# dselivanov/rsparse

Hardware: AMD Instinct MI355X
Metric: als_iterations_per_sec (higher is better)
Workload: dtype f32 (Gram products of rows > 512 / <= 32 non-zeros as 2 x fp16 / 3 x bf16 split terms of the fp32 operands, fp32 accumulate; everything else fp32); 1 GPU; WRMF implicit ALS, CG(3), synthetic 10000000x1000000, 500155883 nnz, rank 128, lambda 0.1; survey_config=3, feedback=implicit, n_items=1000000, nnz=500155883, rank=128, solver=conjugate_gradient, cg_steps=3, parallelism=rows sharded x1, factors replicated

## Files before the change

rsparse_amd/csrc/wrmf_capi.cpp:

```cpp
#include "../../include/rsparse_wrmf_hip.h"

#include <cxxabi.h>

#include <algorithm>
#include <cfloat>
#include <cmath>
#include <cstdlib>
#include <cstring>
#include <functional>
#include <queue>
#include <string>
#include <vector>

#include "wrmf_internal.h"

using namespace rsparse_hip;

struct rsparse_hip_csc {
  DevCSC d;
  int device = 0;
};

namespace {

// ... 569 lines not shown
    hipError_t we = wave_cg ? launch_wide_cg_wave(a, implicit, kWideCgMaxLen, d.max_len > kWideCgMaxLen ? d.q_order : nullptr, 0, s)
                            : launch_als_wide(a, implicit, solver, g_ws.wide_m2, g_ws.wide_lu, s);
    if (we != hipSuccess) return hip_fail(we, wave_cg ? "launch_wide_cg_wave" : "launch_als_wide");
    if ((we = launch_sum_partials(g_ws.partials, wave_cg ? (size_t)grid_w : (size_t)grid, outw, s, g_ws.partials + g_ws.partial_slots)) != hipSuccess)
      return hip_fail(we, "launch_sum_partials");
    return RSPARSE_HIP_OK;
  }
  const bool cg = solver == RSPARSE_SOLVER_CONJUGATE_GRADIENT;
  const bool cgq = cg && use_cgq(rank, d_X, d_Y);
  QSchedule qs;
  qs.order = d.q_order;
  qs.cfg = d.q_cfg;
  qs.pair_first = d.q_pair_first;
  for (int b = 0; b < 7; b++) qs.off[b] = d.q_off[b];
  qs.team4_first = (implicit && bias && bias->gbias != 0.f) ? d.q_off[2] : d.q_team4_first;
  const bool ne_fine = implicit && padded_rank(rank) == 128;
  qs.ne_rows = ne_fine ? d.q_ne_rows : d.q_ne1_rows; qs.ne_ptr = ne_fine ? d.q_ne_ptr : d.q_ne1_ptr;
  qs.ne_wg = ne_fine ? d.q_ne_wg : d.q_ne1_wg; qs.ne_entries = d.q_ne_entries;
  qs.ne_split_rows = d.q_ne_split_rows; qs.ne_split_ptr = d.q_ne_split_ptr; qs.ne_nsplit = d.q_ne_nsplit;
  const bool cg_mf = cgq && implicit && !bias && cg_mf_supported(rank, implicit) && d.q_order && d.q_off[1] > d.q_n_nec;
  if (cg_mf) {
    qs.ne_rows = d.q_nec_rows; qs.ne_ptr = d.q_nec_ptr; qs.ne_wg = d.q_nec_wg; qs.ne_entries = d.q_nec_entries;
    qs.ne_split_rows = d.q_nec_split_rows; qs.ne_split_ptr = d.q_nec_split_ptr; qs.ne_nsplit = d.q_nec_nsplit;
    qs.mf_rows = d.q_order + d.q_n_nec;
    qs.mf_n = d.q_off[1] - d.q_n_nec;
  }
  const bool chol_mf = chol_mf_supported(rank) && !cg && solver == RSPARSE_SOLVER_CHOLESKY && !bias && d.q_order && ne_supported(rank) &&
                       use_cgq(rank, d_X, d_Y) && d.q_lr_first > d.q_off[1];
  const int mf_first = d.q_off[1];
  const int n_mf = chol_mf ? d.q_lr_first - mf_first : 0;
// ... 1182 lines not shown
```

rsparse_amd/csrc/wrmf_cgp.hip:

```cpp
#include "wrmf_internal.h"
#include "wrmf_device.h"

namespace rsparse_hip {
namespace {

using namespace dev;

typedef float f32x2 __attribute__((ext_vector_type(2)));
typedef float f32x4 __attribute__((ext_vector_type(4)));
typedef _Float16 f16x2 __attribute__((ext_vector_type(2)));
typedef _Float16 f16x8 __attribute__((ext_vector_type(8)));

constexpr float kCgTolP = 1e-10f;
constexpr int kPairMaxSweeps = 4;

__device__ __forceinline__ float p_row16_sum(float v) {
  v += dpp<0xB1>(v);
  v += dpp<0x4E>(v);
  v += dpp<0x141>(v);
  v += dpp<0x140>(v);
  return v;
}
__device__ __forceinline__ float p_row16_max(float v) {
  v = fmaxf(v, dpp<0xB1>(v));
// ... 8 lines not shown
  return __uint_as_float(r[0]) + __uint_as_float(r[1]);
}
__device__ __forceinline__ int p_scale_exp(float vmax) {
  const int eb = (int)((__float_as_uint(vmax) >> 23) & 0xffu);
  return min(253, max(1, 267 - eb));
}
__device__ __forceinline__ void p_split(const float x0, const float x1, unsigned& hi, unsigned& lo) {
  const f32x2 v = {x0, x1};
  const f16x2 h = __builtin_convertvector(v, f16x2);
  const f32x2 r = v - __builtin_convertvector(h, f32x2);
  const f16x2 l = __builtin_convertvector(r, f16x2);
  hi = __builtin_bit_cast(unsigned, h);
  lo = __builtin_bit_cast(unsigned, l);
}

struct PairSmem {
  static constexpr int KP = 128, ps = KP + 8, os = KP + 4;
  static constexpr size_t bytes = (size_t)2 * 8 * ps * 2 + (size_t)8 * os * 4 + (size_t)4 * 64 * 4 + 16;
};

template <bool GB, bool KFULL = false>
__global__ __launch_bounds__(256, 2) void als_cgp_kernel(AlsArgs a, const int32_t* __restrict__ rows, int n_rows, int iters,
                                                        size_t loss_slot0) {
  constexpr int KP = 128, RPN = 8, VW = 4, NV = 2, NQ = 8;
  using SM = PairSmem;
  extern __shared__ __attribute__((aligned(16))) char smem[];
  _Float16* sPh = reinterpret_cast<_Float16*>(smem);
  _Float16* sPl = sPh + 8 * SM::ps;
  float* sOut = reinterpret_cast<float*>(sPl + 8 * SM::ps);
  float* sTsv = sOut + 8 * SM::os;
  const int tid = threadIdx.x, lane = tid & 63, wv = rfl(tid >> 6);
  const int g = lane >> 4, i = lane & 15, H = lane >> 5, g2 = g & 1;
  const int k = KFULL ? KP : a.k;
  const float gbias = GB ? a.gbias : 0.f, ltgt = GB ? a.loss_tgt_const : 1.f;
  for (int e = tid; e < 4 * 64; e += 256) sTsv[e] = 0.f;
  f16x8 gAh[2][4], gAl[2][4];
  float ginv;
  {
    const int m = lane & 15, kb = lane >> 4;
    float gmax = 0.f;
#pragma unroll
    for (int t = 0; t < 2; t++)
#pragma unroll
      for (int ks = 0; ks < 4; ks++)
#pragma unroll
        for (int e = 0; e < 8; e++) {
          const int r = 32 * wv + 16 * t + m, c = 32 * ks + 8 * kb + e;
          {
            const float gv = a.XtX[(size_t)min(r, k - 1) * k + min(c, k - 1)];
            gmax = fmaxf(gmax, fabsf(gv) * ((r < k && c < k) ? 1.f : 0.f));
          }
// ... 5 lines not shown
#pragma unroll
    for (int t = 0; t < 2; t++)
#pragma unroll
      for (int ks = 0; ks < 4; ks++) {
        unsigned hi[4], lo[4];
#pragma unroll
        for (int e = 0; e < 8; e += 2) {
          const int r = 32 * wv + 16 * t + m, c = 32 * ks + 8 * kb + e;
          const float g0v = a.XtX[(size_t)min(r, k - 1) * k + min(c, k - 1)];
          const float g0 = g0v * ((r < k && c < k) ? 1.f : 0.f);
          const float g1v = a.XtX[(size_t)min(r, k - 1) * k + min(c + 1, k - 1)];
          const float g1 = g1v * ((r < k && c + 1 < k) ? 1.f : 0.f);
          p_split(g0 * gs, g1 * gs, hi[e / 2], lo[e / 2]);
        }
        const uint4 h4 = {hi[0], hi[1], hi[2], hi[3]}, l4 = {lo[0], lo[1], lo[2], lo[3]};
        gAh[t][ks] = __builtin_bit_cast(f16x8, h4);
        gAl[t][ks] = __builtin_bit_cast(f16x8, l4);
      }
  }
  __syncthreads();
  float* tacc = sTsv + wv * 64 + 16 * H;
  float* tcur = tacc + 32;
  const int col = 2 * wv + H;
  double wloss = 0.0;
  const int wave_global = blockIdx.x * 4 + wv, total_waves = gridDim.x * 4;
  auto ridx = [&](const int itn) { return (wave_global + itn * total_waves) * 2 + H; };
  int row_c = 0, p1_c = 0, p2_c = 0, row_n = 0;
  if (iters > 0 && ridx(0) < n_rows) {
    row_c = rows[ridx(0)];
    p1_c = a.col_ptrs[row_c];
    p2_c = a.col_ptrs[row_c + 1];
  }
  if (iters > 1 && ridx(1) < n_rows) row_n = rows[ridx(1)];

  int idn[NQ];
  float cvn[NQ], cln = 0.f;
#pragma unroll
  for (int q = 0; q < NQ; q++) {
    idn[q] = 0;
    cvn[q] = 0.f;
  }
  auto request_indices = [&](const bool valid, const int np1, const int ncnt) {
#pragma unroll
    for (int q = 0; q < NQ; q++) {
      const int s = 2 * q + g2;
      const int j = (valid && s < ncnt) ? np1 + s : 0;
      idn[q] = a.row_idx[j];
      cvn[q] = a.vals[j];
    }
    cln = a.vals[(valid && i < ncnt) ? np1 + i : 0];
  };
  auto settle_indices = [&]() {
    asm volatile("" : "+v"(idn[0]), "+v"(idn[1]), "+v"(idn[2]), "+v"(idn[3]), "+v"(idn[4]), "+v"(idn[5]), "+v"(idn[6]), "+v"(idn[7]));
    asm volatile("" : "+v"(cvn[0]), "+v"(cvn[1]), "+v"(cvn[2]), "+v"(cvn[3]), "+v"(cvn[4]), "+v"(cvn[5]), "+v"(cvn[6]), "+v"(cvn[7]), "+v"(cln));
  };
  if constexpr (KFULL) {
    request_indices(iters > 0 && ridx(0) < n_rows, p1_c, p2_c - p1_c);
    settle_indices();
  }

  for (int it = 0; it < iters; ++it) {
    const bool have = ridx(it) < n_rows;
    const int row = have ? row_c : 0, p1 = have ? p1_c : 0, p2 = have ? p2_c : 0;
    {
      int p1_n = 0, p2_n = 0, row_nn = 0;
      if (it + 1 < iters && ridx(it + 1) < n_rows) {
        p1_n = a.col_ptrs[row_n];
        p2_n = a.col_ptrs[row_n + 1];
      }
      if (it + 2 < iters && ridx(it + 2) < n_rows) row_nn = rows[ridx(it + 2)];
      row_c = row_n;
      p1_c = p1_n;
      p2_c = p2_n;
      row_n = row_nn;
    }
    const int cnt = p2 - p1;
    float* yrow = a.Y + (size_t)row * k;
    const bool live = have && (GB || cnt > 0);
    if (have && !live) {
      for (int e = lane & 31; e < k; e += 32) yrow[e] = 0.f;
    }
    const bool blk2 = max(__builtin_amdgcn_readlane(cnt, 0), __builtin_amdgcn_readlane(cnt, 32)) > 8;

    float x[RPN], r[RPN], p[RPN], ap[RPN];
    auto load_warm_start = [&]() {
#pragma unroll
      for (int b = 0; b < NV; b++) {
        const int off = b * 16 * VW + i * VW;
        float4 pc = make_float4(0.f, 0.f, 0.f, 0.f);
        if (have && off < k) pc = *reinterpret_cast<const float4*>(yrow + off);
        const float* pf = reinterpret_cast<const float*>(&pc);
#pragma unroll
        for (int c = 0; c < VW; c++) x[b * VW + c] = pf[c];
      }
    };
    if constexpr (KFULL) load_warm_start();
    float xt[NQ][RPN], cv[NQ];
    {
      int id[NQ];
#pragma unroll
      for (int q = 0; q < NQ; q++) {
        if constexpr (KFULL) {
          id[q] = idn[q];
          cv[q] = cvn[q];
        } else {
          const int s = 2 * q + g2;
          const int j = s < cnt ? p1 + s : 0;
          id[q] = 0;
          cv[q] = 0.f;
          if (q < 4 || blk2) {
            id[q] = a.row_idx[j];
            cv[q] = a.vals[j];
          }
        }
      }
#pragma unroll
      for (int q = 0; q < NQ; q++) {
        const bool in = 2 * q + g2 < cnt;
        id[q] = in ? id[q] : 0;
        cv[q] = in ? cv[q] : 0.f;
      }
#pragma unroll
      for (int q = 0; q < NQ; q++) {
        const bool in = 2 * q + g2 < cnt;
        const float* src = in ? a.X + (size_t)id[q] * k : a.zero_row;
#pragma unroll
        for (int b = 0; b < NV; b++) {
          const int off = b * 16 * VW + i * VW;
          if constexpr (KFULL) {
            float4 pc = make_float4(0.f, 0.f, 0.f, 0.f);
            if (q < 4 || blk2) pc = *reinterpret_cast<const float4*>(src + off);
            const float* pf = reinterpret_cast<const float*>(&pc);
#pragma unroll
            for (int c = 0; c < VW; c++) xt[q][b * VW + c] = pf[c];
          } else {
            float4 pc = make_float4(0.f, 0.f, 0.f, 0.f);
            if (q < 4 || blk2) pc = *reinterpret_cast<const float4*>(src + min(off, k - VW));
            const float* pf = reinterpret_cast<const float*>(&pc);
#pragma unroll
            for (int c = 0; c < VW; c++) xt[q][b * VW + c] = off < k ? pf[c] : 0.f;
          }
        }
      }
    }
    float cl;
    if constexpr (KFULL) cl = (g2 == 0 && i < cnt) ? cln : 0.f;
    else cl = (g2 == 0 && i < cnt) ? a.vals[p1 + i] : 0.f;

    if constexpr (!KFULL) load_warm_start();

    auto sweep = [&](const float(&v)[RPN], const int mode, float(&out)[RPN], float& loss_out) {
      float acc[RPN];
#pragma unroll
      for (int rr = 0; rr < RPN; rr++) acc[rr] = 0.f;
      float vinv = 0.f;
      if (mode != 2) {
        float vmax = 0.f;
#pragma unroll
        for (int rr = 0; rr < RPN; rr++) vmax = fmaxf(vmax, fabsf(v[rr]));
        vmax = p_row16_max(vmax);
        const int ve = p_scale_exp(vmax);
        const float vs = __uint_as_float((unsigned)ve << 23);
// ... 8 lines not shown
          const int off = col * SM::ps + g2 * 16 * VW + i * VW;
          *reinterpret_cast<uint2*>(sPh + off) = make_uint2(h0, h1);
          *reinterpret_cast<uint2*>(sPl + off) = make_uint2(l0, l1);
        }
        __syncthreads();
        f32x4 d0[2], d1[2];
#pragma unroll
        for (int t = 0; t < 2; t++) d0[t] = d1[t] = f32x4{0.f, 0.f, 0.f, 0.f};
        const int nb = (lane & 7) * SM::ps + 8 * (lane >> 4);
#pragma unroll
        for (int ks = 0; ks < 4; ks++) {
          const f16x8 bh = *reinterpret_cast<const f16x8*>(sPh + nb + 32 * ks);
          const f16x8 bl = *reinterpret_cast<const f16x8*>(sPl + nb + 32 * ks);
#pragma unroll
          for (int t = 0; t < 2; t++) {
            d0[t] = __builtin_amdgcn_mfma_f32_16x16x32_f16(gAh[t][ks], bh, d0[t], 0, 0, 0);
            d1[t] = __builtin_amdgcn_mfma_f32_16x16x32_f16(gAh[t][ks], bl, d1[t], 0, 0, 0);
            d1[t] = __builtin_amdgcn_mfma_f32_16x16x32_f16(gAl[t][ks], bh, d1[t], 0, 0, 0);
          }
        }
        if ((lane & 15) < 8) {
#pragma unroll
          for (int t = 0; t < 2; t++) {
            const f32x4 d = (d0[t] + d1[t]) * ginv;
            *reinterpret_cast<f32x4*>(sOut + (lane & 15) * SM::os + 32 * wv + 16 * t + 4 * (lane >> 4)) = d;
          }
        }
      }
      float lacc = 0.f;
      if (mode != 2) {
        float* trec = (mode == 0 ? tacc : tcur) + g2;
#pragma unroll
        for (int q0 = 0; q0 < NQ; q0 += 4) {
          if (q0 == 0 || blk2) {
            float t[4];
            f32x2 s2[4];
#pragma unroll
            for (int u = 0; u < 4; u++) s2[u] = f32x2{0.f, 0.f};
#pragma unroll
            for (int rr = 0; rr < RPN; rr += 2) {
              const f32x2 va = {v[rr], v[rr + 1]};
#pragma unroll
              for (int u = 0; u < 4; u++) {
                const f32x2 xa = {xt[q0 + u][rr], xt[q0 + u][rr + 1]};
                s2[u] = __builtin_elementwise_fma(xa, va, s2[u]);
              }
            }
#pragma unroll
            for (int u = 0; u < 4; u++) t[u] = s2[u].x + s2[u].y;
#pragma unroll
            for (int u = 0; u < 4; u++) t[u] += dpp<0xB1>(t[u]);
#pragma unroll
            for (int u = 0; u < 4; u++) t[u] += dpp<0x4E>(t[u]);
#pragma unroll
            for (int u = 0; u < 4; u++) t[u] += dpp<0x141>(t[u]);
#pragma unroll
            for (int u = 0; u < 4; u++) t[u] += dpp<0x140>(t[u]);
#pragma unroll
            for (int u = 0; u < 4; u++) {
              const int q = q0 + u;
              const float c = cv[q];
              trec[2 * q] = t[u];
              const float w = mode == 0 ? c - (c - 1.f) * (GB ? t[u] + gbias : t[u]) : (c - 1.f) * t[u];
#pragma unroll
              for (int rr = 0; rr < RPN; rr++) acc[rr] = fmaf(w, xt[q][rr], acc[rr]);
            }
          }
        }
      } else {
        wave_sync();
        const float t = tacc[i];
        const float dd = ltgt - t;
        lacc = p_pair_sum(p_row16_sum((g2 == 0 && i < cnt) ? cl * dd * dd : 0.f));
      }
      if (mode != 2) {
        __syncthreads();
        const float f = g2 == 0 ? vinv : 0.f;
#pragma unroll
        for (int b = 0; b < NV; b++) {
          const f32x4 o = *reinterpret_cast<const f32x4*>(sOut + col * SM::os + b * 16 * VW + i * VW);
#pragma unroll
          for (int c = 0; c < VW; c++) acc[b * VW + c] = fmaf(f, o[c], acc[b * VW + c]);
        }
#pragma unroll
        for (int rr = 0; rr < RPN; rr++) out[rr] = p_pair_sum(acc[rr]);
        if constexpr (GB) {
          if (mode == 0) {
#pragma unroll
// ... 8 lines not shown
        }
      } else {
        loss_out = lacc;
      }
    };
    auto dot16 = [&](const float(&u)[RPN], const float(&w)[RPN]) {
      float s = 0.f;
#pragma unroll
      for (int rr = 0; rr < RPN; rr++) s = fmaf(u[rr], w[rr], s);
      return p_row16_sum(s);
    };

    float dummy = 0.f;
    sweep(x, 0, r, dummy);
    if constexpr (KFULL)
      request_indices(it + 1 < iters && ridx(it + 1) < n_rows, p1_c, p2_c - p1_c);
#pragma unroll
    for (int rr = 0; rr < RPN; rr++) p[rr] = r[rr];
    float rsold = dot16(r, r);
    bool conv = !live;
    for (int itc = 0; itc < a.cg_steps; ++itc) {
      sweep(p, 1, ap, dummy);
      const float pap = dot16(p, ap);
      const float alpha = conv ? 0.f : (float)((double)rsold / (double)pap);
      wave_sync();
      if (g2 == 0) tacc[i] = fmaf(alpha, tcur[i], tacc[i]);
      wave_sync();
#pragma unroll
      for (int rr = 0; rr < RPN; rr++) {
        x[rr] = fmaf(alpha, p[rr], x[rr]);
        r[rr] = fmaf(-alpha, ap[rr], r[rr]);
      }
      const float rsnew = dot16(r, r);
      if (!conv) {
        if (rsnew < kCgTolP) {
          conv = true;
        } else {
          const float beta = (float)((double)rsnew / (double)rsold);
#pragma unroll
          for (int rr = 0; rr < RPN; rr++) p[rr] = fmaf(p[rr], beta, r[rr]);
          rsold = rsnew;
// ... 18 lines not shown
#pragma unroll
            for (int c = 0; c < VW; c++) pf[c] = x[b * VW + c];
            *reinterpret_cast<float4*>(yrow + off) = pc;
          }
        }
      }
    }
  }
  const double other = __shfl(wloss, 32);
  if (lane == 0) a.loss_partials[loss_slot0 + (size_t)blockIdx.x * 4 + wv] = wloss + other;
}

}

bool cgp_supported(int k, bool implicit) { return implicit && k > 64 && k <= 128 && k % 4 == 0; }

int cgp_grid(int n_rows) {
  if (n_rows <= 0) return 0;
  const long pairs = ((long)n_rows + 1) / 2;
  long per_wave = 32;
  const long spread = 4L * 512;
  if (pairs < spread * per_wave) per_wave = (pairs + spread - 1) / spread;
  if (per_wave < 1) per_wave = 1;
  return (int)((pairs + 4 * per_wave - 1) / (4 * per_wave));
}

hipError_t launch_als_cgp(const AlsArgs& a, const int32_t* rows, int n_rows, size_t loss_slot0, hipStream_t s,
                          hipEvent_t* ev_slot) {
  const int grid = cgp_grid(n_rows);
  if (grid <= 0) return hipSuccess;
  const long pairs = ((long)n_rows + 1) / 2;
  const int iters = (int)((pairs + (long)grid * 4 - 1) / ((long)grid * 4));
  const bool gb = a.gbias != 0.f;
  auto k0 = als_cgp_kernel<false, false>;
  auto k0f = als_cgp_kernel<false, true>;
  auto k1 = als_cgp_kernel<true, false>;
  const bool full = !gb && a.k == 128;
  const void* fn = gb ? reinterpret_cast<const void*>(k1) : (full ? reinterpret_cast<const void*>(k0f) : reinterpret_cast<const void*>(k0));
  hipError_t err = hipFuncSetAttribute(fn, hipFuncAttributeMaxDynamicSharedMemorySize, (int)PairSmem::bytes);
  if (err != hipSuccess) return err;
  (void)ev_slot;
  if (gb) hipLaunchKernelGGL(k1, dim3(grid), dim3(256), PairSmem::bytes, s, a, rows, n_rows, iters, loss_slot0);
  else if (full) hipLaunchKernelGGL(k0f, dim3(grid), dim3(256), PairSmem::bytes, s, a, rows, n_rows, iters, loss_slot0);
  else hipLaunchKernelGGL(k0, dim3(grid), dim3(256), PairSmem::bytes, s, a, rows, n_rows, iters, loss_slot0);
  return hipGetLastError();
}

}
```

rsparse_amd/csrc/wrmf_cgq.hip:

```cpp
#include <algorithm>

#include "wrmf_internal.h"
#include "wrmf_device.h"

namespace rsparse_hip {
namespace {

using namespace dev;

typedef float f32x2 __attribute__((ext_vector_type(2)));

constexpr int kGvFirstMinCapq = 16;
constexpr int kStreamPrefixQ = 4;
constexpr int kIdxPrefetchMaxWpr = 2;

constexpr float kCgTolQ = 1e-10f;
constexpr int kMaxSavedSweeps = 4;

template <int KP>
struct QG {
  static constexpr int RPN = KP / 16;
  static constexpr int VW = RPN >= 4 ? 4 : RPN;
  static constexpr int NV = RPN / VW;
  __device__ static __forceinline__ int elem(int i, int r) { return (r / VW) * (16 * VW) + i * VW + (r % VW); }
// ... 56 lines not shown
__device__ __forceinline__ void split_f16(const float x0, const float x1, unsigned& hi, unsigned& lo) {
  const f32x2 v = {x0, x1};
  const f16x2 h = __builtin_convertvector(v, f16x2);
  const f32x2 r = v - __builtin_convertvector(h, f32x2);
  const f16x2 l = __builtin_convertvector(r, f16x2);
  hi = __builtin_bit_cast(unsigned, h);
  lo = __builtin_bit_cast(unsigned, l);
}
__device__ __forceinline__ float row16_max(float v) {
  v = fmaxf(v, dpp<0xB1>(v));
  v = fmaxf(v, dpp<0x4E>(v));
  v = fmaxf(v, dpp<0x141>(v));
  v = fmaxf(v, dpp<0x140>(v));
  return v;
}

__device__ __forceinline__ unsigned lds_addr(const void* p) {
  return (unsigned)(reinterpret_cast<uintptr_t>(p));
}
__device__ __forceinline__ void dma4(const void* g, unsigned lds_base) {
  asm volatile("s_mov_b32 m0, %1\n\ts_nop 0\n\tglobal_load_lds_dword %0, off" : : "v"(g), "s"(lds_base) : "memory", "m0");
}
__device__ __forceinline__ void wait_vm0() { asm volatile("s_waitcnt vmcnt(0)" ::: "memory"); }

template <int KP, int CAPQ, int WAVES, int WPR, int STREAM, bool IMPLICIT, int DMF = 0>
struct QSmem {
  static constexpr size_t gram_floats = (IMPLICIT && DMF != 1) ? (size_t)KP * KP : 0;
  static constexpr size_t vec_floats = IMPLICIT ? (size_t)WAVES * KP : 0;
  static constexpr size_t red_floats = WPR > 1 ? (size_t)2 * WAVES * KP + 2 * WAVES : 0;
  static constexpr bool cv_lds = !STREAM && CAPQ * (KP / 16) > 128;
  static constexpr size_t tsv_floats = (STREAM && !IMPLICIT) ? 0 : (size_t)WAVES * (cv_lds ? 3 : 2) * CAPQ * 4;
  static constexpr size_t pre_floats = STREAM ? (size_t)WAVES * kStreamPrefixQ * 4 * KP : 0;
  static constexpr int dmf_ps = KP + 8, dmf_os = KP + 4;
  static constexpr size_t dmf_floats = DMF ? (size_t)WAVES * dmf_ps + (size_t)WAVES * dmf_os : 0;
  static constexpr size_t pfx_floats =
      (!STREAM && WPR > kIdxPrefetchMaxWpr && (CAPQ == 16 || CAPQ == 20)) ? (size_t)WAVES * 2 * CAPQ * 4 : 0;
  static constexpr size_t wl_floats = cv_lds ? (size_t)WAVES * 2 : 0;
  static constexpr size_t xs_floats = cv_lds ? (size_t)WAVES * KP : 0;
// ... 837 lines not shown
};
constexpr int cfg_of_kp(int KP) { return KP == 64 ? 1 : 0; }
constexpr int kTeam4Waves = 4, kTeam4Capq = 20;
static_assert(kTeam4Max == kTeam4Waves * kTeam4Capq * 4, "wrmf_internal.h's split and the kernel's capacity");
constexpr bool team4_split(int KP, bool GB) { return KP == 128 && !GB; }
int team4_first(const QSchedule& q) { return std::min(std::max(q.team4_first, q.off[1]), q.off[2]); }

template <int KP, int WAVES, int CAPQ, int WPR, int STREAM, bool IMPLICIT, bool GB, int DMF = 0, bool KFULL = false>
hipError_t launch_bucket(const AlsArgs& a, const int32_t* rows, int n_rows, int grid, size_t slot0, hipStream_t s,
                         hipEvent_t* ev_slot) {
  if (n_rows <= 0) return hipSuccess;
  constexpr bool kDmfGeometry = IMPLICIT && KP == 128 && WAVES == 4 && WPR == 1 && (CAPQ == 8 || CAPQ == 16) && STREAM == 0;
  if constexpr (kDmfGeometry && !DMF) {
    return launch_bucket<KP, WAVES, CAPQ, WPR, STREAM, IMPLICIT, GB, CAPQ == 8 ? 1 : 2>(a, rows, n_rows, grid, slot0, s, ev_slot);
  } else {
    if constexpr (!KFULL && STREAM == 0) {
      if (a.k == KP)
        return launch_bucket<KP, WAVES, CAPQ, WPR, STREAM, IMPLICIT, GB, DMF, true>(a, rows, n_rows, grid, slot0, s, ev_slot);
    }
    constexpr int TEAMS = WAVES / WPR;
    auto kern = als_cgq_kernel<KP, CAPQ, WAVES, WPR, STREAM, IMPLICIT, DMF, GB, KFULL>;
    const size_t lds = QSmem<KP, CAPQ, WAVES, WPR, STREAM, IMPLICIT, DMF>::bytes;
    hipError_t err = hipFuncSetAttribute(reinterpret_cast<const void*>(kern),
                                         hipFuncAttributeMaxDynamicSharedMemorySize, (int)lds);
    if (err != hipSuccess) return err;
    const int total_teams = grid * TEAMS;
    const int rpt = (n_rows + total_teams - 1) / total_teams;
    prof_note(ev_slot, reinterpret_cast<const void*>(kern));
    hipLaunchKernelGGL(kern, dim3(grid), dim3(WAVES * 64), lds, s, a, rows, n_rows, rpt, slot0);
    return hipGetLastError();
  }
// ... 24 lines not shown
int g_launch_mode = 2;
int concurrent_buckets() { return g_launch_mode; }

size_t bucket_slots(const QSchedule& q, int b, int k, bool implicit) {
  const int cfg = cfg_of_kp(padded_rank(k));
  const BucketDef d = kBuckets[cfg][b];
  if (d.wpr <= 0) return 0;
  if (d.stream && ne_supported(k)) return (size_t)(q.ne_entries + q.ne_nsplit) + (size_t)(q.mf_n > 0 ? cg_mf_loss_slots(q.mf_n) : 0);
  const int rows = q.off[b + 1] - q.off[b];
  if (b == 1 && padded_rank(k) == 128) {
    const int split = team4_first(q);
    return (size_t)cgq_bucket_grid(split - q.off[b], b, cfg) * d.waves + (size_t)cgq_team4_grid(q.off[b + 1] - split) * kTeam4Waves;
  }
  if (b == kNB - 1 && rows > 0 && cgp_supported(k, implicit)) {
    const int split = std::min(std::max(q.pair_first, q.off[b]), q.off[b + 1]);
    return (size_t)cgq_bucket_grid(split - q.off[b], b, cfg) * d.waves + (size_t)cgp_grid(q.off[b + 1] - split) * 4;
  }
  return (size_t)cgq_bucket_grid(rows, b, cfg) * d.waves;
}

template <int KP, int CFG, bool IMPLICIT, bool GB>
hipError_t launch_all(const AlsArgs& a, const QSchedule& q, hipStream_t s, hipEvent_t* ev) {
  hipError_t err;
  size_t slot = 0;
  const int cmode = ev ? 0 : concurrent_buckets();
  const bool overlap = cmode != 0;
  bool forked = false;
  if (overlap) {
    if ((err = g_bs.ensure()) != hipSuccess) return err;
  }
#define RSP_BUCKET(B)                                                                                       \
// ... 43 lines not shown
          return hipErrorInvalidValue;                                                                      \
        } else if constexpr (B == 1 && team4_split(KP, GB)) {                                              \
           \
          const int first = q.off[B], split = team4_first(q);                                               \
          const int n_main = split - first, n_t4 = q.off[B + 1] - split;                                    \
          const int g_main = cgq_bucket_grid(n_main, B, CFG);                                               \
          if ((err = launch_bucket<KP, D.waves, D.capq, D.wpr, D.stream, IMPLICIT, GB>(a, q.order + first, n_main, g_main, slot, \
                                                                                  bs, ev ? ev + B : nullptr)) != hipSuccess) \
            return err;                                                                                     \
          if ((err = launch_bucket<KP, kTeam4Waves, kTeam4Capq, kTeam4Waves, 0, IMPLICIT, GB>(              \
                   a, q.order + split, n_t4, cgq_team4_grid(n_t4), slot + (size_t)g_main * D.waves, bs,     \
                   n_main > 0 ? nullptr : (ev ? ev + B : nullptr))) != hipSuccess)                          \
            return err;                                                                                     \
        } else if (B == kNB - 1 && cgp_supported(a.k, IMPLICIT)) {                    \
           \
          const int first = q.off[B], split = std::min(std::max(q.pair_first, first), q.off[B + 1]);         \
          const int n_main = split - first, n_pair = q.off[B + 1] - split;                                   \
          const int g_main = cgq_bucket_grid(n_main, B, CFG);                                                \
          if ((err = launch_bucket<KP, D.waves, D.capq, D.wpr, D.stream, IMPLICIT, GB>(a, q.order + first, n_main, g_main, slot, \
                                                                                  bs, ev ? ev + B : nullptr)) != hipSuccess) \
            return err;                                                                                     \
          if ((err = launch_als_cgp(a, q.order + split, n_pair, slot + (size_t)g_main * D.waves, bs,          \
                                    n_main > 0 ? nullptr : (ev ? ev + B : nullptr))) != hipSuccess)           \
            return err;                                                                                     \
        } else if ((err = launch_bucket<KP, D.waves, D.capq, D.wpr, D.stream, IMPLICIT, GB>(a, q.order + q.off[B], n, grid, slot, \
                                                                                bs, ev ? ev + B : nullptr)) != hipSuccess) \
          return err;                                                                                       \
        if (side) {                                                                                         \
          if ((err = hipEventRecord(g_bs.done[B], bs)) != hipSuccess) return err;                           \
          if ((err = hipStreamWaitEvent(s, g_bs.done[B], 0)) != hipSuccess) return err;                     \
        }                                                                                                   \
      }                                                                                                     \
      slot += bucket_slots(q, B, a.k, IMPLICIT);                                                             \
    }                                                                                                       \
  }
  RSP_BUCKET(0)
  RSP_BUCKET(1)
// ... 72 lines not shown
```

rsparse_amd/csrc/wrmf_device.h:

```cpp
#pragma once
#include <hip/hip_runtime.h>

namespace rsparse_hip {
namespace dev {

__device__ __forceinline__ void wave_sync() {
  __builtin_amdgcn_fence(__ATOMIC_RELEASE, "wavefront");
  __builtin_amdgcn_wave_barrier();
  __builtin_amdgcn_fence(__ATOMIC_ACQUIRE, "wavefront");
}

__device__ __forceinline__ float readlane_f(float v, int l) {
  return __int_as_float(__builtin_amdgcn_readlane(__float_as_int(v), l));
}
__device__ __forceinline__ int rfl(int v) { return __builtin_amdgcn_readfirstlane(v); }

template <int CTRL>
__device__ __forceinline__ float dpp(float v) {
  return __int_as_float(__builtin_amdgcn_update_dpp(0, __float_as_int(v), CTRL, 0xf, 0xf, true));
}

template <int E>
__device__ __forceinline__ void fnma_row_bcast(float& acc, const float u, const float l) {
  asm("v_fmac_f32_dpp %0, -%1, %2 row_newbcast:%3 row_mask:0xf bank_mask:0xf" : "+v"(acc) : "v"(u), "v"(l), "n"(E));
}
__device__ __forceinline__ void dpp_ready(float& a) { asm("s_nop 1" : "+v"(a)); }
__device__ __forceinline__ void dpp_ready(float& a, float& b) { asm("s_nop 1" : "+v"(a), "+v"(b)); }
__device__ __forceinline__ void dpp_ready(float& a, float& b, float& c, float& d) {
  asm("s_nop 1" : "+v"(a), "+v"(b), "+v"(c), "+v"(d));
}
// ... 156 lines not shown
```

rsparse_amd/csrc/wrmf_internal.h:

```cpp
#pragma once
#include <hip/hip_runtime.h>
#include <cstdint>
#include <string>

namespace rsparse_hip {

struct DevCSC {
  int n_rows = 0;
  int n_cols = 0;
  int64_t nnz = 0;
  const int32_t* col_ptrs = nullptr;
  const int32_t* row_idx = nullptr;
  const float* vals = nullptr;
  int32_t* long_rows = nullptr;
  int n_long = 0;
  int short_max = 0;
  int max_len = 0;
  int32_t* q_order = nullptr;
  int q_off[7] = {0, 0, 0, 0, 0, 0, 0};
  int q_cfg = 0;
  int q_pair_first = 0;
  int q_team4_first = 0;
  int64_t q_nnz[6] = {0, 0, 0, 0, 0, 0};
  int64_t* q_stream_off = nullptr;
// ... 79 lines not shown
  const int32_t* ne_segs;
  float* ne_seg_scratch;
  int* ne_seg_flags;
  int ne_chol;
  int ne_chol_min;
  const unsigned* ne_stats;
  const float* mf_XtX;
  const unsigned* wave_stats;
};

struct QSchedule {
  const int32_t* order;
  int off[7];
  int pair_first;
  int team4_first;
  int cfg;
  const int32_t* ne_rows;
  const int32_t* ne_ptr;
  int ne_wg;
  int ne_entries;
  const int32_t* ne_split_rows;
  const int32_t* ne_split_ptr;
  int ne_nsplit;
  const int32_t* mf_rows = nullptr;
  int mf_n = 0;
};
int cgq_default_cfg();
void cgq_set_launch_mode(int mode);
int cgq_num_buckets();
int cgq_bucket_wpr(int cfg, int b);
int cgq_bucket_capq(int cfg, int b);
int cgq_bucket_waves(int cfg, int b);
int cgq_bucket_stream(int cfg, int b);
int cgq_bucket_grid(int n_rows, int bucket, int cfg);
constexpr int kTeam4Max = 320;
int cgq_team4_grid(int n_rows);
int cgq_bucket_of(int len, int cfg);
size_t cgq_loss_slots(const QSchedule& q, int k, bool implicit);
bool cgp_supported(int k, bool implicit);
int cgp_grid(int n_rows);
hipError_t launch_als_cgp(const AlsArgs& a, const int32_t* rows, int n_rows, size_t loss_slot0, hipStream_t s,
                          hipEvent_t* ev_slot);
bool ne_supported(int k);
constexpr int kNeMinLen = 512;
constexpr int kNeMaxSeg = 16;
constexpr int kNeMaxSegTotal = 1024;
constexpr int kNeSegFloats = 4 * (11 * 16 * 64 + 128 + 2);
hipError_t launch_ne_stats(const float* X, int64_t nx, const float* vals, int64_t nnz, unsigned* stats, hipStream_t s,
                           const float* absmax_hint = nullptr, const unsigned* cached_vstats = nullptr,
                           unsigned* save_vstats = nullptr);
struct QSchedule;
hipError_t launch_als_ne(const AlsArgs& a, const QSchedule& q, bool implicit, double* row_loss, hipStream_t s,
                         hipEvent_t* ev_slot = nullptr);
hipError_t launch_gb_row_terms(const AlsArgs& a, const int32_t* rows, int n, float* out, int32_t* slot_of_row, hipStream_t s);
hipError_t launch_als_cgq(const AlsArgs& a, const QSchedule& q, bool implicit, hipStream_t s, hipEvent_t* ev = nullptr);

// ... 139 lines not shown
```

rsparse_amd/csrc/wrmf_ne.hip:

```cpp
#include <type_traits>
#include <utility>

#include "wrmf_internal.h"
#include "wrmf_device.h"
#include "wrmf_ldlt.h"

namespace rsparse_hip {
namespace {

using namespace dev;

typedef float f32x16 __attribute__((ext_vector_type(16)));
typedef float f32x2 __attribute__((ext_vector_type(2)));
typedef __bf16 bf16x2 __attribute__((ext_vector_type(2)));
typedef __bf16 bf16x8 __attribute__((ext_vector_type(8)));
typedef unsigned u32x4 __attribute__((ext_vector_type(4)));

constexpr float kCgTolNe = 1e-10f;
constexpr int kStepNnz = 16;

struct NeMfmaOp { int slot, m, R, C, pa, pb; };
struct NeUnit { int kind, t, pair; };

template <int KP, int NS, bool IMPLICIT, bool SYM = false, bool QUAD = false>
// ... 110 lines not shown
  static constexpr int GROUP = NI / LOADERS + (LOADERS == 1 ? 2 : 1);
  static constexpr int RING_BYTES = D * SLOT_BYTES + IDXR * 256;
  static constexpr int TLD = 33;
  static constexpr int A_FLOATS = NT * 32 * TLD;
  static constexpr int G_FLOATS = IMPLICIT && !QUAD ? A_FLOATS : 0;
  static constexpr int YB = QUAD ? 4 : 8;
  static constexpr int V_FLOATS = 4 * KP  + 2 * NB * NB * 32  +
                                  4 * KP  + 256  +
                                  YB * KP + 4 * YB  + 64 ;
  static constexpr int BYTES = NRING * RING_BYTES + (A_FLOATS + G_FLOATS + V_FLOATS) * 4;
  static_assert(BYTES <= (QUAD ? 80 : 160) * 1024, "LDS budget");
  static_assert((D - 2) * GROUP <= 63, "vmcnt is a 6-bit field");
  __host__ __device__ static constexpr int tile(int R, int C) { return R * (R + 1) / 2 + C; }
};

__device__ __forceinline__ unsigned lds_addr(const void* p) {
  return (unsigned)(reinterpret_cast<uintptr_t>(p));
}

__device__ __forceinline__ void dma16(const void* g, unsigned lds_base) {
  asm volatile("s_mov_b32 m0, %1\n\ts_nop 0\n\tglobal_load_lds_dwordx4 %0, off" : : "v"(g), "s"(lds_base) : "memory", "m0");
}
__device__ __forceinline__ void dma4(const void* g, unsigned lds_base) {
  asm volatile("s_mov_b32 m0, %1\n\ts_nop 0\n\tglobal_load_lds_dword %0, off" : : "v"(g), "s"(lds_base) : "memory", "m0");
}
template <int N>
__device__ __forceinline__ void wait_vm() {
  asm volatile("s_waitcnt vmcnt(%0)" ::"n"(N) : "memory");
}
__device__ __forceinline__ int sload(const int* p) {
  int v;
  asm volatile("s_load_dword %0, %1, 0x0\n\ts_waitcnt lgkmcnt(0)" : "=s"(v) : "s"(p) : "memory");
  return v;
}

__device__ __forceinline__ unsigned pack_bf16(float lo, float hi) {
  const f32x2 f = {lo, hi};
  const bf16x2 h = __builtin_convertvector(f, bf16x2);
  return __builtin_bit_cast(unsigned, h);
// ... 1111 lines not shown
```

Baseline: 8.291 iterations/s.

## Route last CG bucket's main rows through a 32-slot pair kernel variant

Adds a wide (NQ=16) variant of the pair-CG kernel for rank 128 without global bias. Its Gram fragments move from registers to LDS and the next row's indices and values are prefetched into LDS with global-to-LDS DMA. The scheduler then sends the main rows of the final short-row bucket to this kernel instead of the generic cgq bucket kernel, with loss-slot accounting adjusted to match. This trades register pressure for LDS traffic and a larger LDS footprint per block, which may reduce occupancy. It also disables the KFULL specialization for one DMF cgq path and moves the DMA helpers to a shared header.

```diff
diff --git a/rsparse_amd/csrc/wrmf_capi.cpp b/rsparse_amd/csrc/wrmf_capi.cpp
--- a/rsparse_amd/csrc/wrmf_capi.cpp
+++ b/rsparse_amd/csrc/wrmf_capi.cpp
@@ -607,6 +607,7 @@
   qs.pair_first = d.q_pair_first;
   for (int b = 0; b < 7; b++) qs.off[b] = d.q_off[b];
   qs.team4_first = (implicit && bias && bias->gbias != 0.f) ? d.q_off[2] : d.q_team4_first;
+  qs.pair_wide = cgp_wide_supported(rank, implicit, implicit && bias && bias->gbias != 0.f);
   const bool ne_fine = implicit && padded_rank(rank) == 128;
   qs.ne_rows = ne_fine ? d.q_ne_rows : d.q_ne1_rows; qs.ne_ptr = ne_fine ? d.q_ne_ptr : d.q_ne1_ptr;
   qs.ne_wg = ne_fine ? d.q_ne_wg : d.q_ne1_wg; qs.ne_entries = d.q_ne_entries;
diff --git a/rsparse_amd/csrc/wrmf_cgp.hip b/rsparse_amd/csrc/wrmf_cgp.hip
--- a/rsparse_amd/csrc/wrmf_cgp.hip
+++ b/rsparse_amd/csrc/wrmf_cgp.hip
@@ -46,27 +46,34 @@
   lo = __builtin_bit_cast(unsigned, l);
 }
 
+template <int NQ>
 struct PairSmem {
   static constexpr int KP = 128, ps = KP + 8, os = KP + 4;
-  static constexpr size_t bytes = (size_t)2 * 8 * ps * 2 + (size_t)8 * os * 4 + (size_t)4 * 64 * 4 + 16;
+  static constexpr size_t gfrag = NQ == 16 ? (size_t)4 * 16 * 1024 : 0;
+  static constexpr size_t nxt = NQ == 16 ? (size_t)4 * 2 * 2 * 64 * 4 : 0;
+  static constexpr size_t bytes = gfrag + (size_t)2 * 8 * ps * 2 + (size_t)8 * os * 4 + (size_t)4 * 8 * NQ * 4 + nxt + 16;
 };
 
-template <bool GB, bool KFULL = false>
+template <bool GB, bool KFULL = false, int NQ = 8>
 __global__ __launch_bounds__(256, 2) void als_cgp_kernel(AlsArgs a, const int32_t* __restrict__ rows, int n_rows, int iters,
                                                         size_t loss_slot0) {
-  constexpr int KP = 128, RPN = 8, VW = 4, NV = 2, NQ = 8;
-  using SM = PairSmem;
+  constexpr int KP = 128, RPN = 8, VW = 4, NV = 2;
+  static_assert(NQ == 8 || (NQ == 16 && KFULL && !GB), "the 32-slot kernel: rank 128, no global bias");
+  constexpr bool GREG = NQ == 8;
+  using SM = PairSmem<NQ>;
   extern __shared__ __attribute__((aligned(16))) char smem[];
-  _Float16* sPh = reinterpret_cast<_Float16*>(smem);
+  char* sGf = smem + (size_t)(threadIdx.x >> 6) * 16 * 1024;
+  _Float16* sPh = reinterpret_cast<_Float16*>(smem + SM::gfrag);
   _Float16* sPl = sPh + 8 * SM::ps;
   float* sOut = reinterpret_cast<float*>(sPl + 8 * SM::ps);
   float* sTsv = sOut + 8 * SM::os;
+  float* sNx = sTsv + 4 * 8 * NQ + (threadIdx.x >> 6) * 256;
   const int tid = threadIdx.x, lane = tid & 63, wv = rfl(tid >> 6);
   const int g = lane >> 4, i = lane & 15, H = lane >> 5, g2 = g & 1;
   const int k = KFULL ? KP : a.k;
   const float gbias = GB ? a.gbias : 0.f, ltgt = GB ? a.loss_tgt_const : 1.f;
-  for (int e = tid; e < 4 * 64; e += 256) sTsv[e] = 0.f;
-  f16x8 gAh[2][4], gAl[2][4];
+  for (int e = tid; e < 4 * 8 * NQ; e += 256) sTsv[e] = 0.f;
+  f16x8 gAh[GREG ? 2 : 1][GREG ? 4 : 1], gAl[GREG ? 2 : 1][GREG ? 4 : 1];
   float ginv;
   {
     const int m = lane & 15, kb = lane >> 4;
@@ -102,13 +109,20 @@
           p_split(g0 * gs, g1 * gs, hi[e / 2], lo[e / 2]);
         }
         const uint4 h4 = {hi[0], hi[1], hi[2], hi[3]}, l4 = {lo[0], lo[1], lo[2], lo[3]};
-        gAh[t][ks] = __builtin_bit_cast(f16x8, h4);
-        gAl[t][ks] = __builtin_bit_cast(f16x8, l4);
+        if constexpr (GREG) {
+          gAh[t][ks] = __builtin_bit_cast(f16x8, h4);
+          gAl[t][ks] = __builtin_bit_cast(f16x8, l4);
+        } else {
+          *reinterpret_cast<uint4*>(sGf + ((t * 4 + ks) * 2 + 0) * 1024 + lane * 16) = h4;
+          *reinterpret_cast<uint4*>(sGf + ((t * 4 + ks) * 2 + 1) * 1024 + lane * 16) = l4;
+        }
       }
   }
   __syncthreads();
-  float* tacc = sTsv + wv * 64 + 16 * H;
-  float* tcur = tacc + 32;
+  float* tacc = sTsv + wv * 8 * NQ + 2 * NQ * H;
+  float* tcur = tacc + 4 * NQ;
+  const int lslot = NQ == 16 ? i + 16 * g2 : i;
+  const bool lgrp = NQ == 16 || g2 == 0;
   const int col = 2 * wv + H;
   double wloss = 0.0;
   const int wave_global = blockIdx.x * 4 + wv, total_waves = gridDim.x * 4;
@@ -121,14 +135,22 @@
   }
   if (iters > 1 && ridx(1) < n_rows) row_n = rows[ridx(1)];
 
-  int idn[NQ];
-  float cvn[NQ], cln = 0.f;
-#pragma unroll
-  for (int q = 0; q < NQ; q++) {
+  int idn[GREG ? NQ : 1];
+  float cvn[GREG ? NQ : 1], cln = 0.f;
+#pragma unroll
+  for (int q = 0; q < (GREG ? NQ : 1); q++) {
     idn[q] = 0;
     cvn[q] = 0.f;
   }
-  auto request_indices = [&](const bool valid, const int np1, const int ncnt) {
+  auto request_indices = [&](const bool valid, const int np1, const int ncnt, const int buf) {
+    if constexpr (!GREG) {
+      const int e = lane & 31;
+      const bool in = valid && e < ncnt;
+      float* slot = sNx + buf * 128;
+      dma4(in ? static_cast<const void*>(a.row_idx + np1 + e) : static_cast<const void*>(a.zero_row), (unsigned)rfl((int)lds_addr(slot)));
+      dma4(in ? static_cast<const void*>(a.vals + np1 + e) : static_cast<const void*>(a.zero_row), (unsigned)rfl((int)lds_addr(slot + 64)));
+      return;
+    }
 #pragma unroll
     for (int q = 0; q < NQ; q++) {
       const int s = 2 * q + g2;
@@ -136,14 +158,22 @@
       idn[q] = a.row_idx[j];
       cvn[q] = a.vals[j];
     }
-    cln = a.vals[(valid && i < ncnt) ? np1 + i : 0];
+    cln = a.vals[(valid && lslot < ncnt) ? np1 + lslot : 0];
   };
   auto settle_indices = [&]() {
-    asm volatile("" : "+v"(idn[0]), "+v"(idn[1]), "+v"(idn[2]), "+v"(idn[3]), "+v"(idn[4]), "+v"(idn[5]), "+v"(idn[6]), "+v"(idn[7]));
-    asm volatile("" : "+v"(cvn[0]), "+v"(cvn[1]), "+v"(cvn[2]), "+v"(cvn[3]), "+v"(cvn[4]), "+v"(cvn[5]), "+v"(cvn[6]), "+v"(cvn[7]), "+v"(cln));
+    if constexpr (!GREG) {
+      wait_vm0();
+      return;
+    }
+#pragma unroll
+    for (int q = 0; q < NQ; q += 8) {
+      asm volatile("" : "+v"(idn[q]), "+v"(idn[q + 1]), "+v"(idn[q + 2]), "+v"(idn[q + 3]), "+v"(idn[q + 4]), "+v"(idn[q + 5]), "+v"(idn[q + 6]), "+v"(idn[q + 7]));
+      asm volatile("" : "+v"(cvn[q]), "+v"(cvn[q + 1]), "+v"(cvn[q + 2]), "+v"(cvn[q + 3]), "+v"(cvn[q + 4]), "+v"(cvn[q + 5]), "+v"(cvn[q + 6]), "+v"(cvn[q + 7]));
+    }
+    asm volatile("" : "+v"(cln));
   };
   if constexpr (KFULL) {
-    request_indices(iters > 0 && ridx(0) < n_rows, p1_c, p2_c - p1_c);
+    request_indices(iters > 0 && ridx(0) < n_rows, p1_c, p2_c - p1_c, 0);
     settle_indices();
   }
 
@@ -168,7 +198,8 @@
     if (have && !live) {
       for (int e = lane & 31; e < k; e += 32) yrow[e] = 0.f;
     }
-    const bool blk2 = max(__builtin_amdgcn_readlane(cnt, 0), __builtin_amdgcn_readlane(cnt, 32)) > 8;
+    const int wcnt = max(__builtin_amdgcn_readlane(cnt, 0), __builtin_amdgcn_readlane(cnt, 32));
+    auto blk_on = [&](const int q) { return q < 4 || wcnt > 2 * (q & ~3); };
 
     float x[RPN], r[RPN], p[RPN], ap[RPN];
     auto load_warm_start = [&]() {
@@ -183,12 +214,15 @@
       }
     };
     if constexpr (KFULL) load_warm_start();
-    float xt[NQ][RPN], cv[NQ];
+    float xt[NQ][RPN], cv[GREG ? NQ : 1];
+    const float* nx = sNx + (it & 1) * 128 + 32 * H;
     {
       int id[NQ];
 #pragma unroll
       for (int q = 0; q < NQ; q++) {
-        if constexpr (KFULL) {
+        if constexpr (!GREG) {
+          id[q] = __float_as_int(nx[2 * q + g2]);
+        } else if constexpr (KFULL) {
           id[q] = idn[q];
           cv[q] = cvn[q];
         } else {
@@ -196,7 +230,7 @@
           const int j = s < cnt ? p1 + s : 0;
           id[q] = 0;
           cv[q] = 0.f;
-          if (q < 4 || blk2) {
+          if (blk_on(q)) {
             id[q] = a.row_idx[j];
             cv[q] = a.vals[j];
           }
@@ -206,7 +240,7 @@
       for (int q = 0; q < NQ; q++) {
         const bool in = 2 * q + g2 < cnt;
         id[q] = in ? id[q] : 0;
-        cv[q] = in ? cv[q] : 0.f;
+        if constexpr (GREG) cv[q] = in ? cv[q] : 0.f;
       }
 #pragma unroll
       for (int q = 0; q < NQ; q++) {
@@ -217,13 +251,13 @@
           const int off = b * 16 * VW + i * VW;
           if constexpr (KFULL) {
             float4 pc = make_float4(0.f, 0.f, 0.f, 0.f);
-            if (q < 4 || blk2) pc = *reinterpret_cast<const float4*>(src + off);
+            if (blk_on(q)) pc = *reinterpret_cast<const float4*>(src + off);
             const float* pf = reinterpret_cast<const float*>(&pc);
 #pragma unroll
             for (int c = 0; c < VW; c++) xt[q][b * VW + c] = pf[c];
           } else {
             float4 pc = make_float4(0.f, 0.f, 0.f, 0.f);
-            if (q < 4 || blk2) pc = *reinterpret_cast<const float4*>(src + min(off, k - VW));
+            if (blk_on(q)) pc = *reinterpret_cast<const float4*>(src + min(off, k - VW));
             const float* pf = reinterpret_cast<const float*>(&pc);
 #pragma unroll
             for (int c = 0; c < VW; c++) xt[q][b * VW + c] = off < k ? pf[c] : 0.f;
@@ -232,8 +266,9 @@
       }
     }
     float cl;
-    if constexpr (KFULL) cl = (g2 == 0 && i < cnt) ? cln : 0.f;
-    else cl = (g2 == 0 && i < cnt) ? a.vals[p1 + i] : 0.f;
+    if constexpr (!GREG) cl = nx[64 + lslot];
+    else if constexpr (KFULL) cl = (lgrp && lslot < cnt) ? cln : 0.f;
+    else cl = (lgrp && lslot < cnt) ? a.vals[p1 + lslot] : 0.f;
 
     if constexpr (!KFULL) load_warm_start();
 
@@ -272,9 +307,17 @@
           const f16x8 bl = *reinterpret_cast<const f16x8*>(sPl + nb + 32 * ks);
 #pragma unroll
           for (int t = 0; t < 2; t++) {
-            d0[t] = __builtin_amdgcn_mfma_f32_16x16x32_f16(gAh[t][ks], bh, d0[t], 0, 0, 0);
-            d1[t] = __builtin_amdgcn_mfma_f32_16x16x32_f16(gAh[t][ks], bl, d1[t], 0, 0, 0);
-            d1[t] = __builtin_amdgcn_mfma_f32_16x16x32_f16(gAl[t][ks], bh, d1[t], 0, 0, 0);
+            f16x8 ah, al;
+            if constexpr (GREG) {
+              ah = gAh[t][ks];
+              al = gAl[t][ks];
+            } else {
+              ah = *reinterpret_cast<const f16x8*>(sGf + ((t * 4 + ks) * 2 + 0) * 1024 + lane * 16);
+              al = *reinterpret_cast<const f16x8*>(sGf + ((t * 4 + ks) * 2 + 1) * 1024 + lane * 16);
+            }
+            d0[t] = __builtin_amdgcn_mfma_f32_16x16x32_f16(ah, bh, d0[t], 0, 0, 0);
+            d1[t] = __builtin_amdgcn_mfma_f32_16x16x32_f16(ah, bl, d1[t], 0, 0, 0);
+            d1[t] = __builtin_amdgcn_mfma_f32_16x16x32_f16(al, bh, d1[t], 0, 0, 0);
           }
         }
         if ((lane & 15) < 8) {
@@ -290,7 +333,7 @@
         float* trec = (mode == 0 ? tacc : tcur) + g2;
 #pragma unroll
         for (int q0 = 0; q0 < NQ; q0 += 4) {
-          if (q0 == 0 || blk2) {
+          if (blk_on(q0)) {
             float t[4];
             f32x2 s2[4];
 #pragma unroll
@@ -317,7 +360,7 @@
 #pragma unroll
             for (int u = 0; u < 4; u++) {
               const int q = q0 + u;
-              const float c = cv[q];
+              const float c = GREG ? cv[q] : nx[64 + 2 * q + g2];
               trec[2 * q] = t[u];
               const float w = mode == 0 ? c - (c - 1.f) * (GB ? t[u] + gbias : t[u]) : (c - 1.f) * t[u];
 #pragma unroll
@@ -327,9 +370,9 @@
         }
       } else {
         wave_sync();
-        const float t = tacc[i];
+        const float t = tacc[lslot];
         const float dd = ltgt - t;
-        lacc = p_pair_sum(p_row16_sum((g2 == 0 && i < cnt) ? cl * dd * dd : 0.f));
+        lacc = p_pair_sum(p_row16_sum((lgrp && lslot < cnt) ? cl * dd * dd : 0.f));
       }
       if (mode != 2) {
         __syncthreads();
@@ -368,7 +411,7 @@
     float dummy = 0.f;
     sweep(x, 0, r, dummy);
     if constexpr (KFULL)
-      request_indices(it + 1 < iters && ridx(it + 1) < n_rows, p1_c, p2_c - p1_c);
+      request_indices(it + 1 < iters && ridx(it + 1) < n_rows, p1_c, p2_c - p1_c, (it + 1) & 1);
 #pragma unroll
     for (int rr = 0; rr < RPN; rr++) p[rr] = r[rr];
     float rsold = dot16(r, r);
@@ -378,7 +421,7 @@
       const float pap = dot16(p, ap);
       const float alpha = conv ? 0.f : (float)((double)rsold / (double)pap);
       wave_sync();
-      if (g2 == 0) tacc[i] = fmaf(alpha, tcur[i], tacc[i]);
+      if (lgrp) tacc[lslot] = fmaf(alpha, tcur[lslot], tacc[lslot]);
       wave_sync();
 #pragma unroll
       for (int rr = 0; rr < RPN; rr++) {
@@ -427,6 +470,7 @@
 }
 
 bool cgp_supported(int k, bool implicit) { return implicit && k > 64 && k <= 128 && k % 4 == 0; }
+bool cgp_wide_supported(int k, bool implicit, bool gbias) { return implicit && k == 128 && !gbias; }
 
 int cgp_grid(int n_rows) {
   if (n_rows <= 0) return 0;
@@ -438,24 +482,29 @@
   return (int)((pairs + 4 * per_wave - 1) / (4 * per_wave));
 }
 
-hipError_t launch_als_cgp(const AlsArgs& a, const int32_t* rows, int n_rows, size_t loss_slot0, hipStream_t s,
+hipError_t launch_als_cgp(const AlsArgs& a, const int32_t* rows, int n_rows, bool wide, size_t loss_slot0, hipStream_t s,
                           hipEvent_t* ev_slot) {
   const int grid = cgp_grid(n_rows);
   if (grid <= 0) return hipSuccess;
   const long pairs = ((long)n_rows + 1) / 2;
   const int iters = (int)((pairs + (long)grid * 4 - 1) / ((long)grid * 4));
   const bool gb = a.gbias != 0.f;
+  const bool full = !gb && a.k == 128;
+  if (wide && !full) return hipErrorInvalidValue;
   auto k0 = als_cgp_kernel<false, false>;
   auto k0f = als_cgp_kernel<false, true>;
   auto k1 = als_cgp_kernel<true, false>;
-  const bool full = !gb && a.k == 128;
-  const void* fn = gb ? reinterpret_cast<const void*>(k1) : (full ? reinterpret_cast<const void*>(k0f) : reinterpret_cast<const void*>(k0));
-  hipError_t err = hipFuncSetAttribute(fn, hipFuncAttributeMaxDynamicSharedMemorySize, (int)PairSmem::bytes);
+  auto kw = als_cgp_kernel<false, true, 16>;
+  const void* fn = wide ? reinterpret_cast<const void*>(kw)
+                        : gb ? reinterpret_cast<const void*>(k1) : (full ? reinterpret_cast<const void*>(k0f) : reinterpret_cast<const void*>(k0));
+  const size_t lds = wide ? PairSmem<16>::bytes : PairSmem<8>::bytes;
+  hipError_t err = hipFuncSetAttribute(fn, hipFuncAttributeMaxDynamicSharedMemorySize, (int)lds);
   if (err != hipSuccess) return err;
-  (void)ev_slot;
-  if (gb) hipLaunchKernelGGL(k1, dim3(grid), dim3(256), PairSmem::bytes, s, a, rows, n_rows, iters, loss_slot0);
-  else if (full) hipLaunchKernelGGL(k0f, dim3(grid), dim3(256), PairSmem::bytes, s, a, rows, n_rows, iters, loss_slot0);
-  else hipLaunchKernelGGL(k0, dim3(grid), dim3(256), PairSmem::bytes, s, a, rows, n_rows, iters, loss_slot0);
+  prof_note(ev_slot, fn);
+  if (wide) hipLaunchKernelGGL(kw, dim3(grid), dim3(256), lds, s, a, rows, n_rows, iters, loss_slot0);
+  else if (gb) hipLaunchKernelGGL(k1, dim3(grid), dim3(256), lds, s, a, rows, n_rows, iters, loss_slot0);
+  else if (full) hipLaunchKernelGGL(k0f, dim3(grid), dim3(256), lds, s, a, rows, n_rows, iters, loss_slot0);
+  else hipLaunchKernelGGL(k0, dim3(grid), dim3(256), lds, s, a, rows, n_rows, iters, loss_slot0);
   return hipGetLastError();
 }
 
diff --git a/rsparse_amd/csrc/wrmf_cgq.hip b/rsparse_amd/csrc/wrmf_cgq.hip
--- a/rsparse_amd/csrc/wrmf_cgq.hip
+++ b/rsparse_amd/csrc/wrmf_cgq.hip
@@ -94,14 +94,6 @@
   v = fmaxf(v, dpp<0x140>(v));
   return v;
 }
-
-__device__ __forceinline__ unsigned lds_addr(const void* p) {
-  return (unsigned)(reinterpret_cast<uintptr_t>(p));
-}
-__device__ __forceinline__ void dma4(const void* g, unsigned lds_base) {
-  asm volatile("s_mov_b32 m0, %1\n\ts_nop 0\n\tglobal_load_lds_dword %0, off" : : "v"(g), "s"(lds_base) : "memory", "m0");
-}
-__device__ __forceinline__ void wait_vm0() { asm volatile("s_waitcnt vmcnt(0)" ::: "memory"); }
 
 template <int KP, int CAPQ, int WAVES, int WPR, int STREAM, bool IMPLICIT, int DMF = 0>
 struct QSmem {
@@ -969,7 +961,7 @@
   if constexpr (kDmfGeometry && !DMF) {
     return launch_bucket<KP, WAVES, CAPQ, WPR, STREAM, IMPLICIT, GB, CAPQ == 8 ? 1 : 2>(a, rows, n_rows, grid, slot0, s, ev_slot);
   } else {
-    if constexpr (!KFULL && STREAM == 0) {
+    if constexpr (!KFULL && STREAM == 0 && !(DMF == 1 && !GB)) {
       if (a.k == KP)
         return launch_bucket<KP, WAVES, CAPQ, WPR, STREAM, IMPLICIT, GB, DMF, true>(a, rows, n_rows, grid, slot0, s, ev_slot);
     }
@@ -1024,7 +1016,8 @@
   }
   if (b == kNB - 1 && rows > 0 && cgp_supported(k, implicit)) {
     const int split = std::min(std::max(q.pair_first, q.off[b]), q.off[b + 1]);
-    return (size_t)cgq_bucket_grid(split - q.off[b], b, cfg) * d.waves + (size_t)cgp_grid(q.off[b + 1] - split) * 4;
+    const size_t main = q.pair_wide ? (size_t)cgp_grid(split - q.off[b]) * 4 : (size_t)cgq_bucket_grid(split - q.off[b], b, cfg) * d.waves;
+    return main + (size_t)cgp_grid(q.off[b + 1] - split) * 4;
   }
   return (size_t)cgq_bucket_grid(rows, b, cfg) * d.waves;
 }
@@ -1098,13 +1091,22 @@
             return err;                                                                                     \
         } else if (B == kNB - 1 && cgp_supported(a.k, IMPLICIT)) {                    \
            \
+                                                 \
           const int first = q.off[B], split = std::min(std::max(q.pair_first, first), q.off[B + 1]);         \
           const int n_main = split - first, n_pair = q.off[B + 1] - split;                                   \
-          const int g_main = cgq_bucket_grid(n_main, B, CFG);                                                \
-          if ((err = launch_bucket<KP, D.waves, D.capq, D.wpr, D.stream, IMPLICIT, GB>(a, q.order + first, n_main, g_main, slot, \
-                                                                                  bs, ev ? ev + B : nullptr)) != hipSuccess) \
-            return err;                                                                                     \
-          if ((err = launch_als_cgp(a, q.order + split, n_pair, slot + (size_t)g_main * D.waves, bs,          \
+          size_t main_slots;                                                                                \
+          if (q.pair_wide) {                                                                                \
+            if ((err = launch_als_cgp(a, q.order + first, n_main, true, slot, bs, ev ? ev + B : nullptr)) != hipSuccess) \
+              return err;                                                                                   \
+            main_slots = (size_t)cgp_grid(n_main) * 4;                                                      \
+          } else {                                                                                          \
+            const int g_main = cgq_bucket_grid(n_main, B, CFG);                                             \
+            if ((err = launch_bucket<KP, D.waves, D.capq, D.wpr, D.stream, IMPLICIT, GB>(a, q.order + first, n_main, g_main, slot, \
+                                                                                    bs, ev ? ev + B : nullptr)) != hipSuccess) \
+              return err;                                                                                   \
+            main_slots = (size_t)g_main * D.waves;                                                          \
+          }                                                                                                 \
+          if ((err = launch_als_cgp(a, q.order + split, n_pair, false, slot + main_slots, bs,               \
                                     n_main > 0 ? nullptr : (ev ? ev + B : nullptr))) != hipSuccess)           \
             return err;                                                                                     \
         } else if ((err = launch_bucket<KP, D.waves, D.capq, D.wpr, D.stream, IMPLICIT, GB>(a, q.order + q.off[B], n, grid, slot, \
diff --git a/rsparse_amd/csrc/wrmf_device.h b/rsparse_amd/csrc/wrmf_device.h
--- a/rsparse_amd/csrc/wrmf_device.h
+++ b/rsparse_amd/csrc/wrmf_device.h
@@ -14,6 +14,14 @@
   return __int_as_float(__builtin_amdgcn_readlane(__float_as_int(v), l));
 }
 __device__ __forceinline__ int rfl(int v) { return __builtin_amdgcn_readfirstlane(v); }
+
+__device__ __forceinline__ unsigned lds_addr(const void* p) {
+  return (unsigned)(reinterpret_cast<uintptr_t>(p));
+}
+__device__ __forceinline__ void dma4(const void* g, unsigned lds_base) {
+  asm volatile("s_mov_b32 m0, %1\n\ts_nop 0\n\tglobal_load_lds_dword %0, off" : : "v"(g), "s"(lds_base) : "memory", "m0");
+}
+__device__ __forceinline__ void wait_vm0() { asm volatile("s_waitcnt vmcnt(0)" ::: "memory"); }
 
 template <int CTRL>
 __device__ __forceinline__ float dpp(float v) {
diff --git a/rsparse_amd/csrc/wrmf_internal.h b/rsparse_amd/csrc/wrmf_internal.h
--- a/rsparse_amd/csrc/wrmf_internal.h
+++ b/rsparse_amd/csrc/wrmf_internal.h
@@ -117,6 +117,7 @@
   int off[7];
   int pair_first;
   int team4_first;
+  bool pair_wide;
   int cfg;
   const int32_t* ne_rows;
   const int32_t* ne_ptr;
@@ -141,8 +142,9 @@
 int cgq_bucket_of(int len, int cfg);
 size_t cgq_loss_slots(const QSchedule& q, int k, bool implicit);
 bool cgp_supported(int k, bool implicit);
+bool cgp_wide_supported(int k, bool implicit, bool gbias);
 int cgp_grid(int n_rows);
-hipError_t launch_als_cgp(const AlsArgs& a, const int32_t* rows, int n_rows, size_t loss_slot0, hipStream_t s,
+hipError_t launch_als_cgp(const AlsArgs& a, const int32_t* rows, int n_rows, bool wide, size_t loss_slot0, hipStream_t s,
                           hipEvent_t* ev_slot);
 bool ne_supported(int k);
 constexpr int kNeMinLen = 512;
diff --git a/rsparse_amd/csrc/wrmf_ne.hip b/rsparse_amd/csrc/wrmf_ne.hip
--- a/rsparse_amd/csrc/wrmf_ne.hip
+++ b/rsparse_amd/csrc/wrmf_ne.hip
@@ -148,15 +148,8 @@
   __host__ __device__ static constexpr int tile(int R, int C) { return R * (R + 1) / 2 + C; }
 };
 
-__device__ __forceinline__ unsigned lds_addr(const void* p) {
-  return (unsigned)(reinterpret_cast<uintptr_t>(p));
-}
-
 __device__ __forceinline__ void dma16(const void* g, unsigned lds_base) {
   asm volatile("s_mov_b32 m0, %1\n\ts_nop 0\n\tglobal_load_lds_dwordx4 %0, off" : : "v"(g), "s"(lds_base) : "memory", "m0");
-}
-__device__ __forceinline__ void dma4(const void* g, unsigned lds_base) {
-  asm volatile("s_mov_b32 m0, %1\n\ts_nop 0\n\tglobal_load_lds_dword %0, off" : : "v"(g), "s"(lds_base) : "memory", "m0");
 }
 template <int N>
 __device__ __forceinline__ void wait_vm() {
```

Result: faster. 8.445 iterations/s, median of 6 (+1.9%).
